# IanYeung/RealVSR

Hardware: AMD Instinct MI355X
Metric: HR frames/sec (fwd+bwd) on 5-frame 180x320 LR windows (higher is better)
Workload: dtype f32 (bf16x3 GEMM); 1 GPU; EDVR-M nf64, 5-frame 180x320 LR windows, batch 8 per GPU, x4 output, VideoSRModel.optimize_parameters: fwd + LapPyr(ssim,cb) on Y + GWLoss on CbCr + bwd + Adam step; per_gpu_batch=8, global_batch=8, parallelism=sequence-dp1, gemm=bf16x3 (3-term bf16 split on v_mfma_f32_32x32x16_bf16, f32 accumulate), lf_term=ssim (restated IQA_pytorch.SSIM, parity unpinned)

## Files before the change

include/realvsr_hip.h:

```cpp
#ifndef REALVSR_HIP_H
#define REALVSR_HIP_H
#include <stddef.h>
#ifdef __cplusplus
extern "C" {
#endif

#define RVSR_OK 0
#define RVSR_ERR_UNSUPPORTED 1
#define RVSR_ERR_BAD_ARG 2
#define RVSR_ERR_LAUNCH 3
#define RVSR_ERR_WORKSPACE 4

const char* rvsr_last_error(void);

void rvsr_set_gemm_mode(int mode);
int rvsr_get_gemm_mode(void);
void rvsr_set_gemm_mode_thread(int mode);


size_t rvsr_modulated_deform_conv_forward_workspace_bytes(int channels, int channels_out);
int rvsr_modulated_deform_conv_forward(const float* input, const float* weight, const float* bias,
                                       const float* offset, const float* mask, float* output,
                                       int batch, int channels, int height, int width, int channels_out,
                                       int kernel_h, int kernel_w, int stride_h, int stride_w,
// ... 44 lines not shown
int rvsr_dcn_pack_forward_plan(const float* input, const float* weight, const float* bias, const float* om,
                               float* output, int batch, int channels, int height, int width, int channels_out,
                               int stride, int pad, int dilation, int deformable_group, int act, float slope,
                               void* probe, void* workspace, size_t workspace_bytes, long long* plan);
int rvsr_dcn_pack_backward_plan(const float* input, const float* weight, const float* om, const float* grad_output,
                                const float* act_out, float act_slope, float* grad_input, float* grad_weight,
                                float* grad_bias, float* grad_om, int batch, int channels, int height, int width,
                                int channels_out, int stride, int pad, int dilation, int deformable_group,
                                const void* probe, void* workspace, size_t workspace_bytes, long long* plan);
int rvsr_dcn_fused_takes(int batch, int channels, int height, int width, int channels_out, int kernel_h, int kernel_w, int stride_h,
                         int stride_w, int pad_h, int pad_w, int dilation_h, int dilation_w, int group, int deformable_group);
size_t rvsr_dcn_probe_samples(int batch, int deformable_group, int height_out, int width_out);
int rvsr_dcn_forward_halo(const unsigned* counters, size_t nsamples, int channels_out);

size_t rvsr_deform_conv_generic_workspace_bytes(int dtype, int channels, int height, int width, int kernel_h, int kernel_w,
                                                int stride_h, int stride_w, int pad_h, int pad_w, int dilation_h, int dilation_w);
size_t rvsr_deform_conv_generic_forward_workspace_bytes(int dtype, int channels, int height, int width, int kernel_h, int kernel_w,
                                                        int stride_h, int stride_w, int pad_h, int pad_w, int dilation_h,
                                                        int dilation_w);
int rvsr_deform_conv_generic_forward(int dtype, const void* input, const void* weight, const void* bias, const void* offset,
                                     const void* mask, void* output, int batch, int channels, int height, int width,
                                     int channels_out, int kernel_h, int kernel_w, int stride_h, int stride_w, int pad_h, int pad_w,
                                     int dilation_h, int dilation_w, int group, int deformable_group, void* workspace,
                                     size_t workspace_bytes, void* stream);
int rvsr_deform_conv_generic_backward(int dtype, const void* input, const void* weight, const void* offset, const void* mask,
                                      const void* grad_output, void* grad_input, void* grad_offset, void* grad_mask,
                                      void* grad_weight, void* grad_bias, int batch, int channels, int height, int width,
                                      int channels_out, int kernel_h, int kernel_w, int stride_h, int stride_w, int pad_h, int pad_w,
                                      int dilation_h, int dilation_w, int group, int deformable_group, void* workspace,
                                      size_t workspace_bytes, void* stream);


size_t rvsr_conv2d_forward_workspace_bytes(int C1, int C2, int Co, int ksize);
int rvsr_conv2d_forward(const float* x1, int C1, const float* x2, int C2, const float* xact, float xact_slope,
                        int in_mode, int Hs, int Ws, const float* weight, const float* bias,
                        const float* residual, float* out1, int Co1, float* out2, int Co2, int B, int ksize,
                        int stride, int w_mode, int act, float slope, int pixel_shuffle, int Hout, int Wout,
                        void* workspace, size_t workspace_bytes, void* stream);
int rvsr_conv2d_forward_plan(const float* x1, int C1, const float* x2, int C2, const float* xact, float xact_slope,
                             int in_mode, int Hs, int Ws, const float* weight, const float* bias,
                             const float* residual, float* out1, int Co1, float* out2, int Co2, int B, int ksize,
                             int stride, int w_mode, int act, float slope, int pixel_shuffle, int Hout, int Wout, int* plan);

size_t rvsr_conv2d_pack_weights(const float* weight, int C_in, int Co, int ksize, int w_mode, void* out, size_t out_bytes,
                                long long* desc, void* stream);
int rvsr_pack_weights_batched(const void* descs, int n, void* stream);

size_t rvsr_conv2d_wgrad_workspace_bytes(int C1, int C2, int Co, int B, int ksize, int stride, int Hout, int Wout);
int rvsr_conv2d_backward_weight(const float* x1, int C1, const float* x2, int C2, int Hin, int Win,
                                const float* gout, const float* gact, float gact_slope, int g_mode,
                                int Gs_h, int Gs_w, float* grad_weight, float* grad_bias, int Co, int B,
                                int ksize, int stride, int Hout, int Wout, int accumulate,
                                void* workspace, size_t workspace_bytes, void* stream);


int rvsr_upsample_bilinear_forward(const float* in, float* out, size_t planes, int H, int W, int factor,
                                   float scale, void* stream);
int rvsr_upsample_bilinear_backward(const float* gout, float* gin, size_t planes, int H, int W, int factor,
                                    float scale, void* stream);

int rvsr_maxavgpool_forward(const float* in, float* out, unsigned char* argmax, int B, int C, int H, int W,
                            void* stream);
int rvsr_maxavgpool_backward(const float* gout, const unsigned char* argmax, float* gin, int B, int C, int H,
                             int W, void* stream);

int rvsr_tsa_temporal_forward(const float* emb, const float* emb_ref, const float* aligned, float* mod,
                              float* prob, int B, int N, int C, int H, int W, int frame_major, void* stream);
int rvsr_tsa_temporal_backward(const float* gmod, const float* emb, const float* emb_ref, const float* aligned,
                               const float* prob, float* galigned, float* gemb, float* gemb_ref, int B, int N,
                               int C, int H, int W, int frame_major, void* stream);

int rvsr_tsa_output_forward(const float* fea, const float* att, const float* att_add, float* out, size_t n,
                            void* stream);
int rvsr_tsa_output_backward(const float* g, const float* fea, const float* att, float* gfea, float* gatt,
                             size_t n, void* stream);


int rvsr_pyr_down_forward(const float* in, float* out, size_t planes, int H, int W, void* stream);
int rvsr_pyr_down_backward(const float* gout, float* gin, size_t planes, int H, int W, void* stream);
int rvsr_pyr_updiff_forward(const float* cur, const float* down, float* out, size_t planes, int H, int W,
                            void* stream);
int rvsr_pyr_updiff_backward(const float* gout, float* gdown, size_t planes, int H, int W, void* stream);

size_t rvsr_charbonnier_workspace_bytes(void);
int rvsr_charbonnier_forward(const float* x, const float* y, size_t n, float eps, double scale, float* out,
                             void* workspace, void* stream);
int rvsr_charbonnier_backward(const float* x, const float* y, const float* gscalar, float scale, float eps,
                              float* gx, size_t n, void* stream);

int rvsr_gwloss_forward(const float* x1, const float* x2, size_t planes, int H, int W, float w, double scale, float* out,
                        float* fa, float* fbx, float* fby, void* workspace, void* stream);
int rvsr_gwloss_backward(const float* fa, const float* fbx, const float* fby, const float* gscalar, float scale, float* gx,
                         size_t planes, int H, int W, void* stream);


int rvsr_ycbcr_to_bgr_u8(const float* ycc, unsigned char* bgr, int H, int W, void* stream);


size_t rvsr_reduce_workspace_bytes(void);

int rvsr_pixel_loss_forward(const float* x, const float* y, size_t n, int mode, float param, double scale, float* out,
                            void* workspace, void* stream);
int rvsr_pixel_loss_backward(const float* x, const float* y, const float* gscalar, int mode, float param, float scale,
                             float* gx, size_t n, void* stream);

int rvsr_ssim_forward(const float* x, const float* y, size_t planes, int H, int W, double scale, float* out, float* ga,
// ... 41 lines not shown
```

realvsr_amd/_lib.py:

```python
import ctypes
import os
import subprocess

import torch

_CSRC = os.path.join(os.path.dirname(os.path.abspath(__file__)), 'csrc')
SO_PATH = os.environ.get('RVSR_SO', os.path.join(_CSRC, 'librealvsr_hip.so'))
_lib = None

c_fp = ctypes.c_void_p
c_int, c_float, c_double, c_size = ctypes.c_int, ctypes.c_float, ctypes.c_double, ctypes.c_size_t

_CONV_CALL = [c_fp, c_int, c_fp, c_int, c_fp, c_float, c_int, c_int, c_int, c_fp, c_fp, c_fp, c_fp, c_int, c_fp, c_int, c_int, c_int,
              c_int, c_int, c_int, c_float, c_int, c_int, c_int]
SIGNATURES = {
    'rvsr_last_error': (ctypes.c_char_p, []),
    'rvsr_modulated_deform_conv_forward': (c_int, [c_fp] * 6 + [c_int] * 16 + [c_fp, c_size, c_fp]),
    'rvsr_modulated_deform_conv_forward_workspace_bytes': (c_size, [c_int] * 2),
    'rvsr_modulated_deform_conv_backward_workspace_bytes': (c_size, [c_int] * 8),
    'rvsr_modulated_deform_conv_backward': (c_int, [c_fp] * 11 + [c_int] * 16 + [c_fp, c_size, c_fp]),
    'rvsr_deform_conv_workspace_bytes': (c_size, [c_int] * 11),
    'rvsr_deform_conv_forward': (c_int, [c_fp] * 4 + [c_int] * 16 + [c_fp, c_size, c_fp]),
    'rvsr_deform_conv_backward_input': (c_int, [c_fp] * 6 + [c_int] * 16 + [c_fp, c_size, c_fp]),
    'rvsr_deform_conv_backward_parameters': (c_int, [c_fp] * 4 + [c_int] * 15 + [c_float, c_int, c_fp, c_size, c_fp]),
    'rvsr_deform_conv_generic_workspace_bytes': (c_size, [c_int] * 12),
    'rvsr_deform_conv_generic_forward_workspace_bytes': (c_size, [c_int] * 12),
    'rvsr_deform_conv_generic_forward': (c_int, [c_int] + [c_fp] * 6 + [c_int] * 15 + [c_fp, c_size, c_fp]),
    'rvsr_deform_conv_generic_backward': (c_int, [c_int] + [c_fp] * 10 + [c_int] * 15 + [c_fp, c_size, c_fp]),
    'rvsr_dcn_pack_forward': (c_int, [c_fp] * 5 + [c_int] * 10 + [c_float, c_fp, c_fp, c_size, c_fp]),
    'rvsr_dcn_offset_probe': (c_int, [c_fp, c_int, c_int, c_int, c_int, c_fp, c_fp]),
    'rvsr_dcn_pack_backward': (c_int, [c_fp] * 5 + [c_float] + [c_fp] * 4 + [c_int] * 9 + [c_fp, c_fp, c_size, c_fp]),
    'rvsr_dcn_pack_forward_plan': (c_int, [c_fp] * 5 + [c_int] * 10 + [c_float, c_fp, c_fp, c_size, ctypes.POINTER(ctypes.c_longlong)]),
    'rvsr_dcn_pack_backward_plan': (c_int, [c_fp] * 5 + [c_float] + [c_fp] * 4 + [c_int] * 9 + [c_fp, c_fp, c_size,
                                                                                             ctypes.POINTER(ctypes.c_longlong)]),
    'rvsr_dcn_fused_takes': (c_int, [c_int] * 15),
    'rvsr_dcn_probe_samples': (c_size, [c_int] * 4),
    'rvsr_dcn_forward_halo': (c_int, [c_fp, c_size, c_int]),
    'rvsr_conv2d_forward': (c_int, _CONV_CALL + [c_fp, c_size, c_fp]),
    'rvsr_conv2d_forward_plan': (c_int, _CONV_CALL + [ctypes.POINTER(c_int)]),
    'rvsr_conv2d_forward_workspace_bytes': (c_size, [c_int] * 4),
    'rvsr_conv2d_pack_weights': (c_size, [c_fp, c_int, c_int, c_int, c_int, c_fp, c_size, ctypes.POINTER(ctypes.c_longlong), c_fp]),
    'rvsr_dcn_pack_weights': (c_size, [c_fp, c_int, c_int, c_fp, c_size, ctypes.POINTER(ctypes.c_longlong), c_fp]),
    'rvsr_pack_weights_batched': (c_int, [c_fp, c_int, c_fp]),
    'rvsr_set_gemm_mode': (None, [c_int]),
    'rvsr_get_gemm_mode': (c_int, []),
    'rvsr_set_gemm_mode_thread': (None, [c_int]),
    'rvsr_conv2d_wgrad_workspace_bytes': (c_size, [c_int] * 8),
    'rvsr_conv2d_backward_weight': (c_int, [c_fp, c_int, c_fp, c_int, c_int, c_int, c_fp, c_fp, c_float, c_int, c_int,
                                            c_int, c_fp, c_fp, c_int, c_int, c_int, c_int, c_int, c_int, c_int, c_fp,
                                            c_size, c_fp]),
    'rvsr_upsample_bilinear_forward': (c_int, [c_fp, c_fp, c_size, c_int, c_int, c_int, c_float, c_fp]),
    'rvsr_upsample_bilinear_backward': (c_int, [c_fp, c_fp, c_size, c_int, c_int, c_int, c_float, c_fp]),
    'rvsr_maxavgpool_forward': (c_int, [c_fp, c_fp, c_fp, c_int, c_int, c_int, c_int, c_fp]),
    'rvsr_maxavgpool_backward': (c_int, [c_fp, c_fp, c_fp, c_int, c_int, c_int, c_int, c_fp]),
    'rvsr_tsa_temporal_forward': (c_int, [c_fp] * 5 + [c_int] * 6 + [c_fp]),
    'rvsr_tsa_temporal_backward': (c_int, [c_fp] * 8 + [c_int] * 6 + [c_fp]),
    'rvsr_tsa_output_forward': (c_int, [c_fp] * 4 + [c_size, c_fp]),
    'rvsr_tsa_output_backward': (c_int, [c_fp] * 5 + [c_size, c_fp]),
    'rvsr_pyr_down_forward': (c_int, [c_fp, c_fp, c_size, c_int, c_int, c_fp]),
    'rvsr_pyr_down_backward': (c_int, [c_fp, c_fp, c_size, c_int, c_int, c_fp]),
    'rvsr_pyr_updiff_forward': (c_int, [c_fp, c_fp, c_fp, c_size, c_int, c_int, c_fp]),
    'rvsr_pyr_updiff_backward': (c_int, [c_fp, c_fp, c_size, c_int, c_int, c_fp]),
    'rvsr_charbonnier_workspace_bytes': (c_size, []),
    'rvsr_charbonnier_forward': (c_int, [c_fp, c_fp, c_size, c_float, c_double, c_fp, c_fp, c_fp]),
    'rvsr_charbonnier_backward': (c_int, [c_fp, c_fp, c_fp, c_float, c_float, c_fp, c_size, c_fp]),
    'rvsr_gwloss_forward': (c_int, [c_fp, c_fp, c_size, c_int, c_int, c_float, c_double, c_fp, c_fp, c_fp, c_fp, c_fp, c_fp]),
    'rvsr_gwloss_backward': (c_int, [c_fp, c_fp, c_fp, c_fp, c_float, c_fp, c_size, c_int, c_int, c_fp]),
    'rvsr_ycbcr_to_bgr_u8': (c_int, [c_fp, c_fp, c_int, c_int, c_fp]),
    'rvsr_reduce_workspace_bytes': (c_size, []),
    'rvsr_pixel_loss_forward': (c_int, [c_fp, c_fp, c_size, c_int, c_float, c_double, c_fp, c_fp, c_fp]),
    'rvsr_pixel_loss_backward': (c_int, [c_fp, c_fp, c_fp, c_int, c_float, c_float, c_fp, c_size, c_fp]),
    'rvsr_ssim_forward': (c_int, [c_fp, c_fp, c_size, c_int, c_int, c_double, c_fp, c_fp, c_fp, c_fp, c_fp, c_fp]),
    'rvsr_ssim_backward': (c_int, [c_fp] * 6 + [c_float, c_fp, c_size, c_int, c_int, c_fp]),
    'rvsr_conv_gauss_forward': (c_int, [c_fp, c_fp, c_size, c_int, c_int, c_float, c_fp]),
    'rvsr_conv_gauss_backward': (c_int, [c_fp, c_fp, c_size, c_int, c_int, c_float, c_fp]),
    'rvsr_pyr_upsample_forward': (c_int, [c_fp, c_fp, c_size, c_int, c_int, c_fp]),
    'rvsr_pyr_upsample_backward': (c_int, [c_fp, c_fp, c_size, c_int, c_int, c_fp]),
    'rvsr_adam_step': (c_int, [c_fp] * 4 + [c_size] + [c_float] * 6 + [c_fp]),
    'rvsr_bcast_add_act': (c_int, [c_fp, c_fp, c_size, c_int, c_int, c_float, c_fp]),
    'rvsr_bcast_reduce_act': (c_int, [c_fp, c_fp, c_fp, c_size, c_int, c_float, c_fp]),
    'rvsr_augment_clips': (c_int, [c_fp] * 5 + [c_size] + [c_int] * 10 + [c_float, c_fp]),
    'rvsr_bn_workspace_bytes': (c_size, [c_int] * 3),
    'rvsr_bn_lrelu_forward': (c_int, [c_fp] * 9 + [c_int] * 4 + [c_float] * 3 + [c_fp, c_size, c_fp]),
    'rvsr_bn_lrelu_backward': (c_int, [c_fp] * 9 + [c_int] * 4 + [c_float, c_fp, c_size, c_fp]),
    'rvsr_gan_loss_forward': (c_int, [c_fp, c_size, c_fp, c_size, c_float, c_double, c_fp, c_fp, c_fp]),
    'rvsr_gan_loss_backward': (c_int, [c_fp, c_size, c_size, c_fp, c_fp, c_float, c_float, c_fp, c_fp, c_fp]),
    'rvsr_debug_mfma_rate': (c_int, [c_fp, c_fp, c_int, c_int, c_fp]),
}


def _p(t):
    return None if t is None else ctypes.c_void_p(t.data_ptr())


def _stream():
    return ctypes.c_void_p(torch.cuda.current_stream().cuda_stream)


def build(verbose=False):
    cmd = ['make', '-C', _CSRC, '-j4'] + ([] if verbose else ['-s'])
    subprocess.check_call(cmd)
    if not os.path.exists(SO_PATH):
        raise RuntimeError('build did not produce %s' % SO_PATH)
# ... 57 lines not shown
```

realvsr_amd/csrc/conv2_kernels.hip:

```cpp
#define RVSR_DEFINE_PACK
#include "conv_plan.h"

#include "bf16x3.h"

#ifdef RVSR_ABL5
constexpr int ABL5 = RVSR_ABL5;
#else
constexpr int ABL5 = 0;
#endif

#ifdef RVSR_TIMELINE
__device__ unsigned long long rvsr_dbg[512];
extern "C" int rvsr_debug_read(unsigned long long* out) { return (int)hipMemcpyFromSymbol(out, HIP_SYMBOL(rvsr_dbg), sizeof(unsigned long long) * 512); }
#define STAMP(i) do { if (blockIdx.x == 77 && tid == 0) rvsr_dbg[(i)] = __builtin_amdgcn_s_memtime(); } while (0)
#else
#define STAMP(i) do {} while (0)
#endif

template <int MT, int MODE>
__device__ __forceinline__ void conv2_epilogue(f32x16 (&acc)[MT][2], const ConvFwdParams& p, const float* bias_s, int b,
                                               int o0, int row0, int col, int hi) {
    const float neg = p.act == 0 ? 1.f : (p.act == 1 ? 0.f : p.slope);
    const bool col_ok = col < p.Wout;
    const size_t HW = (size_t)p.Hout * p.Wout;
// ... 1301 lines not shown
            g4[2 * s2] = *reinterpret_cast<const float4*>(gp + pc);
            g4[2 * s2 + 1] = *reinterpret_cast<const float4*>(gp + pc + 4);
            x4[2 * s2] = *reinterpret_cast<const float4*>(xp + pc);
            x4[2 * s2 + 1] = *reinterpret_cast<const float4*>(xp + pc + 4);
            if (ACT) {
                a4[2 * s2] = *reinterpret_cast<const float4*>(ap + pc);
                a4[2 * s2 + 1] = *reinterpret_cast<const float4*>(ap + pc + 4);
            }
        }
#pragma unroll
        for (int s2 = 0; s2 < 2; ++s2) {
            float gv[8] = {g4[2 * s2].x, g4[2 * s2].y, g4[2 * s2].z, g4[2 * s2].w,
                           g4[2 * s2 + 1].x, g4[2 * s2 + 1].y, g4[2 * s2 + 1].z, g4[2 * s2 + 1].w};
            float xv[8] = {x4[2 * s2].x, x4[2 * s2].y, x4[2 * s2].z, x4[2 * s2].w,
                           x4[2 * s2 + 1].x, x4[2 * s2 + 1].y, x4[2 * s2 + 1].z, x4[2 * s2 + 1].w};
            if (ACT) {
                const float av[8] = {a4[2 * s2].x, a4[2 * s2].y, a4[2 * s2].z, a4[2 * s2].w,
                                     a4[2 * s2 + 1].x, a4[2 * s2 + 1].y, a4[2 * s2 + 1].z, a4[2 * s2 + 1].w};
#pragma unroll
                for (int j = 0; j < 8; ++j) gv[j] *= av[j] > 0.f ? 1.f : p.g.slope;
            }
            const bool gok = pv[s2] && o_ok, xok = pv[s2] && c_ok;
#pragma unroll
            for (int j = 0; j < 8; ++j) {
                gv[j] = gok ? gv[j] : 0.f;
                xv[j] = xok ? xv[j] : 0.f;
                bsum += gv[j];
            }
            bf16x8 gh, gl, xh, xl;
            split8(gv, gh, gl);
            split8(xv, xh, xl);
            acc = mfma_bf16(gh, xh, acc);
            acc = mfma_bf16(gh, xl, acc);
            acc = mfma_bf16(gl, xh, acc);
        }
    }
    float* part = p.part + (size_t)blockIdx.x * p.Co * Ctot;
#pragma unroll
    for (int r = 0; r < 16; ++r) {
        const int orow = blockIdx.y * 64 + m * 32 + drow(r, hi);
        if (orow < p.Co && c_ok) part[(size_t)orow * Ctot + c] = acc[r];
    }
    if (p.bpart != nullptr && blockIdx.z == 0 && n == 0) {
        bsum += __shfl_xor(bsum, 32);
        if (hi == 0 && o_ok) p.bpart[(size_t)blockIdx.x * p.Co + o] = bsum;
    }
}

int rvsr_launch_conv_wgrad1x1(const ConvWgradParams& p, int gy, int gz, hipStream_t st) {
    auto k = p.g.act != nullptr ? conv_wgrad1x1_kernel<true> : conv_wgrad1x1_kernel<false>;
    return rvsr_conv_launch("conv_wgrad1x1", k, dim3(p.P, gy, gz), 256, 0, st, p);
}

template <bool ACT>
__global__ __launch_bounds__(256, 2) void conv_wgrad_s2_kernel(const ConvWgradParams p) {
    const int tid = threadIdx.x, lane = tid & 63, wave = tid >> 6, lo = lane & 31, hi = lane >> 5;
    const int m = wave & 1, n = wave >> 1;
    const int C = p.x.a.C;
    const int Hin = p.x.a.Hs, Win = p.x.a.Ws;
    const int Ho = p.Hout, Wo = p.Wout;
    const int o = blockIdx.y * 64 + m * 32 + lo;
    const int c = blockIdx.z * 64 + n * 32 + lo;
    const bool o_ok = o < p.Co, c_ok = c < C;
    const int oc = o_ok ? o : 0, cc = c_ok ? c : 0;
    const int UW = (Wo + 15) / 16;
    const long units = (long)p.B * Ho * UW;
    const long per = (units + p.P - 1) / p.P;
    long u0 = (long)blockIdx.x * per, u1 = u0 + per;
    if (u1 > units) u1 = units;
    f32x16 acc[9];
#pragma unroll
    for (int t = 0; t < 9; ++t) acc[t] = zero16();
    float bsum = 0.f;
    for (long u = u0; u < u1; ++u) {
        const int b = (int)(u / ((long)Ho * UW));
        const int rem = (int)(u - (long)b * Ho * UW);
        const int py = rem / UW, px0 = (rem - py * UW) * 16 + 8 * hi;
        const bool pv = px0 < Wo;
        const size_t gidx = (((size_t)b * p.Co + oc) * Ho + py) * Wo + (pv ? px0 : 0);
        const float4 g0 = *reinterpret_cast<const float4*>(p.g.p + gidx), g1 = *reinterpret_cast<const float4*>(p.g.p + gidx + 4);
        float4 a0, a1;
        if (ACT) {
            a0 = *reinterpret_cast<const float4*>(p.g.act + gidx);
            a1 = *reinterpret_cast<const float4*>(p.g.act + gidx + 4);
        }
        float xr[3][20];
#pragma unroll
        for (int dy = 0; dy < 3; ++dy) {
            const int iy = 2 * py + dy - 1;
            const bool rok = pv && c_ok && iy >= 0 && iy < Hin;
            const float* row = p.x.a.p + (((size_t)b * C + cc) * Hin + (rok ? iy : 0)) * Win;
#pragma unroll
            for (int j = 0; j < 5; ++j) {
                const int col = 2 * px0 - 4 + 4 * j;
                const bool ok = rok && col >= 0 && col < Win;
                const float4 q = *reinterpret_cast<const float4*>(row + (ok ? col : 0));
                xr[dy][4 * j + 0] = ok ? q.x : 0.f; xr[dy][4 * j + 1] = ok ? q.y : 0.f;
                xr[dy][4 * j + 2] = ok ? q.z : 0.f; xr[dy][4 * j + 3] = ok ? q.w : 0.f;
            }
        }
        float gv[8] = {g0.x, g0.y, g0.z, g0.w, g1.x, g1.y, g1.z, g1.w};
        if (ACT) {
            const float av[8] = {a0.x, a0.y, a0.z, a0.w, a1.x, a1.y, a1.z, a1.w};
#pragma unroll
            for (int j = 0; j < 8; ++j) gv[j] *= av[j] > 0.f ? 1.f : p.g.slope;
        }
// ... 148 lines not shown
```

realvsr_amd/csrc/conv_common.h:

```cpp
#pragma once
#include "rvsr_common.h"

struct ConvFwdParams {
    TCat in;
    const float* w;
    const void* wpack;
    int swz;
    int vec4;
    const float* bias;
    const float* res;
    float* out1;
    float* out2;
    int Co1;
    int B, Co, Hout, Wout;
    int w_mode;
    int prepacked;
    int fmt;
    int act;
    float slope;
    int ps;
    int ntx;
};


// ... 16 lines not shown
            for (int r = 0; r < 16; ++r) {
                const int o = o0 + m * 32 + 4 * hi + (r & 3) + 8 * (r >> 2);
                const bool ok = col_ok && o < p.Co;
                const int oc = ok ? o : 0;
                float v = acc[m][n][r];
                const float bb = bp[oc];
                v += has_bias ? bb : 0.f;
                v = v > 0.f ? v : v * neg;
                if (MODE == 3) {
                    const size_t idx = (((size_t)b * (p.Co >> 2) + (oc >> 2)) * (2 * p.Hout) + 2 * row + ((oc >> 1) & 1)) *
                                           (2 * p.Wout) + 2 * col + (oc & 1);
                    if (ok) p.out1[idx] = v;
                } else if (MODE == 2) {
                    const bool first = oc < p.Co1;
                    float* dst = first ? p.out1 : p.out2;
                    const size_t idx = ((size_t)b * (first ? p.Co1 : p.Co - p.Co1) + (first ? oc : oc - p.Co1)) * HW + pix;
                    if (ok) dst[idx] = v;
                } else {
                    const size_t idx = ((size_t)b * p.Co + oc) * HW + pix;
                    if (ok) {
                        if (MODE == 1) v += p.res[idx];
                        p.out1[idx] = v;
                    }
                }
            }
        }
    }
}


struct ConvWgradParams {
    TCat x;
    TView g;
    float* part;
    float* bpart;
    int B, Co, Hout, Wout, ntx, nty, P;
    int ring;
};


struct ConvFwdPlan;
template <typename K, typename P>
static inline int rvsr_conv_launch(const char* name, K k, dim3 grid, unsigned threads, size_t lds, hipStream_t st, const P& p) {
    if (set_lds(k, lds)) FAIL(RVSR_ERR_LAUNCH, "%s: cannot reserve %zu B of LDS", name, lds);
    hipLaunchKernelGGL(k, grid, dim3(threads), lds, st, p);
    hipError_t e = hipGetLastError();
    if (e != hipSuccess) FAIL(RVSR_ERR_LAUNCH, "%s launch: %s", name, hipGetErrorString(e));
    return RVSR_OK;
}
size_t rvsr_conv_fwd2_workspace_bytes(int ksize, int Co, int Ctot);
int rvsr_launch_conv_fwd2(ConvFwdParams p, const ConvFwdPlan& q, int ksize, int stride, void* workspace, size_t workspace_bytes, hipStream_t st);
int rvsr_launch_conv_wgrad2(const ConvWgradParams& p, int gy, int gz, hipStream_t st);
int rvsr_launch_conv_wgrad1x1(const ConvWgradParams& p, int gy, int gz, hipStream_t st);
int rvsr_launch_conv_wgrad_s2(const ConvWgradParams& p, int gy, int gz, hipStream_t st);
int rvsr_launch_conv_wgrad5(const ConvWgradParams& p, int stride, int gy, int gz, hipStream_t st);
int rvsr_launch_conv_wgrad_thin(const ConvWgradParams& p, hipStream_t st);
int rvsr_launch_conv_fwd_thin(const ConvFwdParams& p, const ConvFwdPlan& q, hipStream_t st);
```

realvsr_amd/csrc/conv_kernels.hip:

```cpp
#include "rvsr_common.h"

#include "conv_plan.h"

template <int KS, int STRIDE, int MT, int CC>
__global__ __launch_bounds__(RVSR_WG, 2) void conv_fwd_kernel(const ConvFwdParams p) {
    constexpr int T = KS * KS, PAD = KS / 2, TH = 8, TW = 32;
    constexpr int IH = (TH - 1) * STRIDE + KS, IW = (TW - 1) * STRIDE + KS;
    constexpr int MP = MT * 32, MPP = MP + 1;
    extern __shared__ __attribute__((aligned(16))) float smem[];
    float* xs = smem;
    float* ws = smem + CC * IH * IW;
    const int tid = threadIdx.x, lane = tid & 63, wave = tid >> 6, lo = lane & 31, hi = lane >> 5;
    const int tx = blockIdx.x % p.ntx, ty = blockIdx.x / p.ntx;
    const int x0 = tx * TW, y0 = ty * TH, mb = blockIdx.y, b = blockIdx.z;
    const int Ctot = p.in.a.C + p.in.b.C;

    f32x16 acc[MT][2];
#pragma unroll
    for (int m = 0; m < MT; ++m) {
        acc[m][0] = zero16();
        acc[m][1] = zero16();
    }

    for (int c0 = 0; c0 < Ctot; c0 += CC) {
// ... 302 lines not shown
                                   const float* bias, const float* residual, float* out1, int Co1, float* out2,
                                   int Co2, int B, int ksize, int stride, int w_mode, int act, float slope,
                                   int pixel_shuffle, int Hout, int Wout, void* workspace, size_t workspace_bytes,
                                   void* stream) {
    ConvFwdParams p;
    const int rc = conv_fwd_params(p, x1, C1, x2, C2, xact, xact_slope, in_mode, Hs, Ws, weight, bias, residual, out1, Co1, out2, Co2, B,
                                   ksize, stride, w_mode, act, slope, pixel_shuffle, Hout, Wout);
    if (rc) return rc;
    const ConvFwdPlan q = conv_fwd_plan(p, ksize, stride, rvsr_gemm_mode_now());
    if (q.rc) return conv_fwd_refuse(q);
    hipStream_t st = (hipStream_t)stream;
    switch (q.family) {
        case CONV_FWD_THIN: return rvsr_launch_conv_fwd_thin(p, q, st);
        case CONV_FWD_F32: return launch_fwd(p, q, ksize, stride, st);
        default: return rvsr_launch_conv_fwd2(p, q, ksize, stride, workspace, workspace_bytes, st);
    }
}
extern "C" int rvsr_conv2d_forward_plan(const float* x1, int C1, const float* x2, int C2, const float* xact,
                                        float xact_slope, int in_mode, int Hs, int Ws, const float* weight,
                                        const float* bias, const float* residual, float* out1, int Co1, float* out2,
                                        int Co2, int B, int ksize, int stride, int w_mode, int act, float slope,
                                        int pixel_shuffle, int Hout, int Wout, int* plan) {
    ConvFwdParams p;
    const int rc = conv_fwd_params(p, x1, C1, x2, C2, xact, xact_slope, in_mode, Hs, Ws, weight, bias, residual, out1, Co1, out2, Co2, B,
                                   ksize, stride, w_mode, act, slope, pixel_shuffle, Hout, Wout);
    if (rc) return rc;
    const ConvFwdPlan q = conv_fwd_plan(p, ksize, stride, rvsr_gemm_mode_now());
    const int row[14] = {q.family, q.mt, q.vec, q.wide, q.nt, q.act_in, q.cc, q.vec4, q.th, q.tw, (int)q.gx, (int)q.gy, (int)q.gz, (int)q.lds};
    for (int i = 0; plan && i < 14; ++i) plan[i] = row[i];
    return q.rc ? conv_fwd_refuse(q) : RVSR_OK;
}

int rvsr_g_gemm_mode = 0;
thread_local int rvsr_t_gemm_mode = -1;
extern "C" void rvsr_set_gemm_mode(int mode) { rvsr_g_gemm_mode = (mode >= 0 && mode <= 3) ? mode : 0; }
extern "C" void rvsr_set_gemm_mode_thread(int mode) { rvsr_t_gemm_mode = (mode >= 0 && mode <= 3) ? mode : -1; }
extern "C" int rvsr_get_gemm_mode() { return rvsr_gemm_mode_now(); }
extern "C" size_t rvsr_conv2d_forward_workspace_bytes(int C1, int C2, int Co, int ksize) {
    return rvsr_conv_fwd2_workspace_bytes(ksize, Co, C1 + C2);
}

extern "C" size_t rvsr_conv2d_wgrad_workspace_bytes(int C1, int C2, int Co, int B, int ksize, int stride, int Hout,
                                                    int Wout) {
    const size_t P = conv_wgrad_max_P(ksize, stride, B, Hout, Wout, Co, C1 + C2);
    return sizeof(float) * P * ((size_t)Co * (C1 + C2) * ksize * ksize + Co);
}

template <int KS, int STRIDE, int CCW>
static int launch_wgrad(const ConvWgradParams& p, int gy, int gz, hipStream_t st) {
    constexpr int IH = 3 * STRIDE + KS, IW = 31 * STRIDE + KS, CS = (IH * IW) | 1;
    return rvsr_conv_launch("conv_wgrad", conv_wgrad_kernel<KS, STRIDE, CCW>, dim3(p.P, gy, gz), RVSR_WG, sizeof(float) * (128 * 65 + CCW * CS), st, p);
}

extern "C" int rvsr_conv2d_backward_weight(const float* x1, int C1, const float* x2, int C2, int Hin, int Win,
                                           const float* gout, const float* gact, float gact_slope, int g_mode,
                                           int Gs_h, int Gs_w, float* grad_weight, float* grad_bias, int Co, int B,
                                           int ksize, int stride, int Hout, int Wout, int accumulate, void* workspace,
                                           size_t workspace_bytes, void* stream) {
    if (!x1 || !gout || !grad_weight || B <= 0) FAIL(RVSR_ERR_BAD_ARG, "conv2d_backward_weight: null/empty argument");
    if ((x2 == nullptr) != (C2 == 0)) FAIL(RVSR_ERR_BAD_ARG, "conv2d_backward_weight: x2/C2 disagree");
    if (ksize != 1 && ksize != 3 && ksize != 5) FAIL(RVSR_ERR_UNSUPPORTED, "conv2d_backward_weight: kernel size %d", ksize);
    if (stride != 1 && !(stride == 2 && ksize != 1)) FAIL(RVSR_ERR_UNSUPPORTED, "conv2d_backward_weight: stride %d", stride);
    if (g_mode != 0 && g_mode != 2) FAIL(RVSR_ERR_UNSUPPORTED, "conv2d_backward_weight: gradient view mode %d", g_mode);
    const size_t need = rvsr_conv2d_wgrad_workspace_bytes(C1, C2, Co, B, ksize, stride, Hout, Wout);
    if (!workspace || workspace_bytes < need)
        FAIL(RVSR_ERR_WORKSPACE, "conv2d_backward_weight: workspace %zu B < %zu B", workspace_bytes, need);
    ConvWgradParams p;
    make_view(p.x.a, x1, nullptr, 0.f, C1, Hin, Win, 0, 0, 0);
    make_view(p.x.b, x2, nullptr, 0.f, C2, Hin, Win, 0, 0, 0);
    if (make_view(p.g, gout, gact, gact_slope, Co, Gs_h, Gs_w, g_mode, 0, 0) || p.g.Hv != Hout || p.g.Wv != Wout)
        FAIL(RVSR_ERR_BAD_ARG, "conv2d_backward_weight: gradient view %dx%d (mode %d) vs output %dx%d", Gs_h, Gs_w, g_mode,
             Hout, Wout);
    const int pad = ksize / 2;
    if ((Hin + 2 * pad - ksize) / stride + 1 != Hout || (Win + 2 * pad - ksize) / stride + 1 != Wout)
        FAIL(RVSR_ERR_BAD_ARG, "conv2d_backward_weight: input %dx%d does not give output %dx%d", Hin, Win, Hout, Wout);
    p.B = B;
    p.Co = Co;
    p.Hout = Hout;
    p.Wout = Wout;
    p.ntx = (Wout + 31) / 32;
    p.nty = (Hout + 3) / 4;
    p.ring = 0;
    const ConvWgradPlan q = conv_wgrad_plan(p, ksize, stride, rvsr_gemm_mode_now());
    const size_t nw = (size_t)Co * (C1 + C2) * ksize * ksize;
    p.P = q.P;
    p.part = (float*)workspace;
    p.bpart = grad_bias ? p.part + (size_t)p.P * nw : nullptr;
    hipStream_t st = (hipStream_t)stream;
    int rc = RVSR_ERR_UNSUPPORTED;
    switch (q.family) {
        case CONV_WGRAD_THIN: rc = rvsr_launch_conv_wgrad_thin(p, st); break;
        case CONV_WGRAD2: rc = rvsr_launch_conv_wgrad2(p, q.gy, q.gz, st); break;
        case CONV_WGRAD5: rc = rvsr_launch_conv_wgrad5(p, stride, q.gy, q.gz, st); break;
        case CONV_WGRAD_F32_5: rc = stride == 1 ? launch_wgrad<5, 1, 16>(p, q.gy, q.gz, st) : launch_wgrad<5, 2, 16>(p, q.gy, q.gz, st); break;
        case CONV_WGRAD_1X1: rc = rvsr_launch_conv_wgrad1x1(p, q.gy, q.gz, st); break;
        case CONV_WGRAD_F32_3S1: rc = launch_wgrad<3, 1, 64>(p, q.gy, q.gz, st); break;
        case CONV_WGRAD_S2: rc = rvsr_launch_conv_wgrad_s2(p, q.gy, q.gz, st); break;
        case CONV_WGRAD_F32_3S2: rc = launch_wgrad<3, 2, 32>(p, q.gy, q.gz, st); break;
        case CONV_WGRAD_F32_1: rc = launch_wgrad<1, 1, 64>(p, q.gy, q.gz, st); break;
    }
    if (rc) return rc;
    rvsr_launch_reduce(p.part, p.P, nw, grad_weight, accumulate, st, p.bpart, (size_t)Co, grad_bias);
    hipError_t e = hipGetLastError();
    if (e != hipSuccess) FAIL(RVSR_ERR_LAUNCH, "conv_wgrad reduce launch: %s", hipGetErrorString(e));
    return RVSR_OK;
}
```

realvsr_amd/csrc/conv_plan.h:

```cpp
#pragma once
#include "conv_common.h"

static inline bool conv_al16(const void* a, const void* b = nullptr, const void* c = nullptr, const void* d = nullptr) {
    return ((((uintptr_t)a) | ((uintptr_t)b) | ((uintptr_t)c) | ((uintptr_t)d)) & 15) == 0;
}
static inline bool conv_span_ok(size_t H, size_t W, size_t C) { return sizeof(float) * H * W * C < ((size_t)1 << 31); }


enum ConvFwdFamily {
    CONV_FWD_THIN = 0,
    CONV_FWD5 = 1,
    CONV_FWD2 = 2,
    CONV_FWD_F32 = 3,
};

struct ConvFwdPlan {
    int rc;
    const char* msg;
    int family;
    int mt;
    int vec;
    int wide;
    int nt;
    int act_in;
// ... 70 lines not shown
        q.cc = ksize == 1 ? 32 : ksize == 3 ? (stride == 1 ? (wide_m ? 8 : 16) : (wide_m ? 4 : 8)) : (stride == 1 ? (wide_m ? 4 : 8) : 4);
        const int IH = 7 * stride + ksize, IW = 31 * stride + ksize;
        q.lds = sizeof(float) * ((size_t)q.cc * IH * IW + (size_t)T * q.cc * (q.mt * 32 + 1));
        q.gx = (unsigned)(ntx * nty8);
        q.gy = (unsigned)((p.Co + q.mt * 32 - 1) / (q.mt * 32));
        q.gz = (unsigned)p.B;
        return q;
    }
    q.vec4 = (p.Wout % 4 == 0) && conv_al16(p.out1, p.res) && !p.ps && p.out2 == nullptr && conv_span_ok(p.Hout, p.Wout, p.Co);
    q.cc = ccg;
    q.gy = q.gz = 1;
    long items = (long)nmb * p.B;
    if (ksize != 3 || stride != 1) {
        q.family = CONV_FWD2;
        const int IH = 7 * stride + ksize, IW = 31 * stride + ksize;
        q.lds = (size_t)16 * (2 * (2 * ccg) * IH * IW + 2 * T * (2 * ccg) * (q.mt * 32)) + sizeof(float) * q.mt * 32;
        items *= (long)ntx * nty8;
        const int slots = 256 * (q.lds > 80 * 1024 ? 1 : 2);
        q.gx = (unsigned)(items < slots ? items : slots);
        return q;
    }
    q.family = CONV_FWD5;
    const bool al = conv_al16(va.p, va.act, vb.p);
    if (va.mode == 0 && va.Ws % 4 == 0 && va.Wv == va.Ws && al && conv_span_ok(va.Hs, va.Ws, va.C > vb.C ? va.C : vb.C) &&
        (vb.C == 0 || va.C % 16 == 0))
        q.vec = 1;
    else if (va.mode == 2 && vb.C == 0 && va.C % 16 == 0 && va.Wv % 4 == 0 && va.Ws == 2 * va.Wv && va.Hs == 2 * va.Hv && al &&
             conv_span_ok(va.Hs, va.Ws, va.C >> 2))
        q.vec = 2;
    else if (va.mode == 1 && vb.C == 0 && va.Wv % 4 == 0 && va.Wv == 2 * va.Ws && va.Hv <= 2 * va.Hs && va.Ws % 2 == 0 && al &&
             conv_span_ok(va.Hs, va.Ws, va.C))
        q.vec = 3;
    if (p.fmt && (q.vec != 1 || q.act_in))
        return conv_fwd_refusal("conv2d: the f16 + fp8 format needs a plain 16-byte-aligned input view with W % 4 == 0 and no act' tensor");
    const long px_n = (long)((p.Hout + 15) / 16 * 16) * ((p.Wout + 31) / 32 * 32), px_w = (long)((p.Hout + 7) / 8 * 8) * ((p.Wout + 63) / 64 * 64);
    q.wide = q.mt == 2 && q.vec == 1 && q.vec4 && px_w <= px_n;
    if (p.act == 3 && !q.wide) return conv_fwd_refusal(nullptr);
    if (p.fmt) q.nt = 4;
    else if (q.mt == 2 && q.vec != 0) q.nt = gemm_mode == 2 ? 2 : (gemm_mode == 3 ? 1 : 3);
    q.th = q.wide ? 8 : 16;
    q.tw = q.wide ? 64 : 32;
    const int NX = q.wide ? 2 * 10 * 66 : 2 * 18 * 34, WVEC = 9 * 2 * q.mt * 32;
    q.lds = (size_t)16 * (2 * 2 * NX + 2 * 2 * WVEC) + sizeof(float) * 4 * q.mt * 32 + 16;
    items *= (long)((p.Wout + q.tw - 1) / q.tw) * ((p.Hout + q.th - 1) / q.th);
    q.gx = (unsigned)(items < 256 ? items : 256);
    return q;
}

enum ConvWgradFamily {
    CONV_WGRAD_THIN = 0,
    CONV_WGRAD2,
    CONV_WGRAD5,
    CONV_WGRAD_F32_5,
    CONV_WGRAD_1X1,
    CONV_WGRAD_F32_3S1,
    CONV_WGRAD_S2,
    CONV_WGRAD_F32_3S2,
    CONV_WGRAD_F32_1,
    CONV_WGRAD_FAMILIES
};
struct ConvWgradPlan {
    int family, P, gy, gz;
};

static inline bool conv_wgrad_can(int family, int ksize, int stride, int Co) {
    switch (family) {
        case CONV_WGRAD_THIN: return ksize == 3 && stride == 1 && Co <= 4;
        case CONV_WGRAD2: case CONV_WGRAD_F32_3S1: return ksize == 3 && stride == 1;
        case CONV_WGRAD5: case CONV_WGRAD_F32_5: return ksize == 5;
        case CONV_WGRAD_S2: case CONV_WGRAD_F32_3S2: return ksize == 3 && stride == 2;
        default: return ksize == 1;
    }
}
static inline ConvWgradPlan conv_wgrad_slicing(int family, int B, int Hout, int Wout, int Co, int Ctot) {
    const long ntiles = (long)B * ((Hout + 3) / 4) * ((Wout + 31) / 32);
    long units = ntiles, slots = 256;
    int gy = (Co + 63) / 64, gz = (Ctot + 63) / 64;
    switch (family) {
        case CONV_WGRAD_THIN:
            units = (long)B * ((Hout + 3) / 4) * ((Wout + 63) / 64);
            slots = 768;
            gy = gz = 1;
            break;
        case CONV_WGRAD5:
            gy = (Co + 31) / 32;
            gz = (Ctot + 31) / 32;
            break;
        case CONV_WGRAD_F32_5:
            gz = (Ctot + 15) / 16;
            break;
        case CONV_WGRAD_S2:
            units = (long)B * Hout * ((Wout + 15) / 16);
            slots = 512;
            break;
        case CONV_WGRAD_F32_3S2:
            gz = (Ctot + 31) / 32;
            break;
        case CONV_WGRAD_1X1: case CONV_WGRAD_F32_1:
            slots = 1024;
            break;
        default:
            break;
    }
    long P = slots / ((long)gy * gz);
    if (P < 1) P = 1;
    if (P > units) P = units;
    return {family, (int)P, gy, gz};
}
static inline int conv_wgrad_max_P(int ksize, int stride, int B, int Hout, int Wout, int Co, int Ctot) {
    int P = 0;
    for (int f = 0; f < CONV_WGRAD_FAMILIES; ++f)
        if (conv_wgrad_can(f, ksize, stride, Co)) {
            const int Pf = conv_wgrad_slicing(f, B, Hout, Wout, Co, Ctot).P;
            if (Pf > P) P = Pf;
        }
    return P;
}

static inline ConvWgradPlan conv_wgrad_plan(const ConvWgradParams& p, int ksize, int stride, int gemm_mode) {
    const int C1 = p.x.a.C, C2 = p.x.b.C, Ctot = C1 + C2;
    const bool al = conv_al16(p.x.a.p, p.x.b.p, p.g.p, p.g.act), split = gemm_mode != 1, plain_g = p.g.mode == 0;
    const auto takes = [&](int family) {
        switch (family) {
            case CONV_WGRAD_THIN:
                return C2 == 0 && C1 % 16 == 0 && plain_g && p.Wout % 4 == 0 && al && conv_span_ok(p.Hout, p.Wout, C1);
            case CONV_WGRAD2:
                return split && p.Wout % 4 == 0 && al && conv_span_ok(p.Hout, p.Wout, p.Co > Ctot ? p.Co : Ctot) && (C2 == 0 || C1 % 64 == 0);
            case CONV_WGRAD5: return split;
            case CONV_WGRAD_1X1: return split && plain_g && (p.Hout * p.Wout) % 8 == 0 && al;
            case CONV_WGRAD_S2: return split && C2 == 0 && plain_g && p.Wout % 8 == 0 && p.x.a.Ws % 4 == 0 && al;
            default: return true;
        }
    };
    for (int f = 0; f < CONV_WGRAD_FAMILIES; ++f)
        if (conv_wgrad_can(f, ksize, stride, p.Co) && takes(f)) return conv_wgrad_slicing(f, p.B, p.Hout, p.Wout, p.Co, Ctot);
    return {-1, 0, 0, 0};
}
```

Measured before the change: 81.42 HR frames/s.

## Add wide-channel 1x1 weight-gradient kernel with LDS staging and prefetch

Adds a 512-thread 1x1 conv weight-gradient kernel. Each block covers 64 output channels by up to 320 input channels, stages bf16 hi/lo splits of the gradient and input tiles in LDS, and prefetches the next pixel tile through buffer loads while the current one runs bf16x3 MFMAs. It is placed ahead of the existing 1x1 family in the planner, with its own slicing rules, and a plan-query API is exposed. The aim is more reuse of each gradient tile across many input channels and loads hidden behind compute. In exchange, occupancy drops to one block per CU and there are fewer partial slices to reduce.

Result: faster. 82.26 HR frames/s, median of 6 (+1.0%).

```diff
diff --git a/include/realvsr_hip.h b/include/realvsr_hip.h
--- a/include/realvsr_hip.h
+++ b/include/realvsr_hip.h
@@ -120,6 +120,10 @@
                                 int Gs_h, int Gs_w, float* grad_weight, float* grad_bias, int Co, int B,
                                 int ksize, int stride, int Hout, int Wout, int accumulate,
                                 void* workspace, size_t workspace_bytes, void* stream);
+int rvsr_conv2d_backward_weight_plan(const float* x1, int C1, const float* x2, int C2, int Hin, int Win,
+                                     const float* gout, const float* gact, float gact_slope, int g_mode,
+                                     int Gs_h, int Gs_w, float* grad_weight, int Co, int B, int ksize, int stride,
+                                     int Hout, int Wout, int* plan);
 
 
 int rvsr_upsample_bilinear_forward(const float* in, float* out, size_t planes, int H, int W, int factor,
diff --git a/realvsr_amd/_lib.py b/realvsr_amd/_lib.py
--- a/realvsr_amd/_lib.py
+++ b/realvsr_amd/_lib.py
@@ -49,6 +49,8 @@
     'rvsr_conv2d_backward_weight': (c_int, [c_fp, c_int, c_fp, c_int, c_int, c_int, c_fp, c_fp, c_float, c_int, c_int,
                                             c_int, c_fp, c_fp, c_int, c_int, c_int, c_int, c_int, c_int, c_int, c_fp,
                                             c_size, c_fp]),
+    'rvsr_conv2d_backward_weight_plan': (c_int, [c_fp, c_int, c_fp, c_int, c_int, c_int, c_fp, c_fp, c_float, c_int, c_int, c_int, c_fp] +
+                                         [c_int] * 6 + [ctypes.POINTER(c_int)]),
     'rvsr_upsample_bilinear_forward': (c_int, [c_fp, c_fp, c_size, c_int, c_int, c_int, c_float, c_fp]),
     'rvsr_upsample_bilinear_backward': (c_int, [c_fp, c_fp, c_size, c_int, c_int, c_int, c_float, c_fp]),
     'rvsr_maxavgpool_forward': (c_int, [c_fp, c_fp, c_fp, c_int, c_int, c_int, c_int, c_fp]),
diff --git a/realvsr_amd/csrc/conv2_kernels.hip b/realvsr_amd/csrc/conv2_kernels.hip
--- a/realvsr_amd/csrc/conv2_kernels.hip
+++ b/realvsr_amd/csrc/conv2_kernels.hip
@@ -1377,6 +1377,158 @@
     return rvsr_conv_launch("conv_wgrad1x1", k, dim3(p.P, gy, gz), 256, 0, st, p);
 }
 
+#define WG1_THREADS 512
+#define WG1_KT 64
+#define WG1_CB 320
+#define WG1_RP 144
+#define WG1_ROWS (64 + WG1_CB)
+template <bool ACT>
+__global__ __launch_bounds__(WG1_THREADS, 1) void conv_wgrad1x1s_kernel(const ConvWgradParams p) {
+    extern __shared__ __attribute__((aligned(16))) unsigned char smem_raw[];
+    unsigned char* t_hi = smem_raw;
+    unsigned char* t_lo = smem_raw + WG1_ROWS * WG1_RP;
+    const int tid = threadIdx.x, lane = tid & 63, wave = tid >> 6, lo = lane & 31, hi = lane >> 5;
+    const int m = wave & 1, ng = wave >> 1;
+    const int C1 = p.x.a.C, C2 = p.x.b.C, Ctot = C1 + C2;
+    const int HW = p.Hout * p.Wout;
+    const int o0 = blockIdx.y * 64, c0 = blockIdx.z * WG1_CB;
+    const int cb = Ctot - c0 < WG1_CB ? Ctot - c0 : WG1_CB;
+    const int nblk = (cb + 63) / 64, ntile = (cb + 31) / 32;
+    const bool m_live = o0 + m * 32 < p.Co;
+    const bool do_bias = p.bpart != nullptr && blockIdx.z == 0;
+
+    constexpr int NXI = WG1_CB / 64;
+    constexpr unsigned OOB = 0x80000000u;
+    const int q = tid & 7, r64 = tid >> 3;
+    const unsigned g_vo = o0 + r64 < p.Co ? 4u * (unsigned)((o0 + r64) * HW + 8 * q) : OOB;
+    unsigned x_vo[NXI];
+#pragma unroll
+    for (int i = 0; i < NXI; ++i) {
+        const int c = c0 + 64 * i + r64;
+        x_vo[i] = c < Ctot ? 4u * (unsigned)((c >= C1 ? c - C1 : c) * HW + 8 * q) : OOB;
+    }
+    const size_t img_g = (size_t)p.Co * HW, img_x1 = (size_t)C1 * HW, img_x2 = (size_t)C2 * HW;
+
+    typedef float f32x4v __attribute__((ext_vector_type(4)));
+    auto ld4 = [&](__amdgpu_buffer_rsrc_t rs, unsigned vo, unsigned so) {
+        const f32x4v v = __builtin_bit_cast(f32x4v, __builtin_amdgcn_raw_buffer_load_b128(rs, (int)vo, (int)so, 0));
+        return make_float4(v.x, v.y, v.z, v.w);
+    };
+    float4 gv[2], sv[ACT ? 2 : 1], xv[NXI][2];
+    float bacc = 0.f;
+
+    const int U = (HW + WG1_KT - 1) / WG1_KT;
+    const int ntiles = p.B * U;
+    const int per = (ntiles + p.P - 1) / p.P;
+    const int t_begin = blockIdx.x * per, t_end = t_begin + per < ntiles ? t_begin + per : ntiles;
+
+    auto issue_loads = [&](int tile, int part) {
+        int b = tile / U;
+        int px0 = (tile - b * U) * WG1_KT;
+        asm volatile("" : "+s"(b), "+s"(px0));
+        const int left = HW - px0;
+        const unsigned so = 4u * (unsigned)px0;
+        if (part < 0 || part == 0) {
+            const __amdgpu_buffer_rsrc_t g_rs = buf_view_2g(p.g.p + (size_t)b * img_g);
+            const __amdgpu_buffer_rsrc_t s_rs = buf_view_2g(ACT ? p.g.act + (size_t)b * img_g : p.g.p);
+#pragma unroll
+            for (int kk = 0; kk < 2; ++kk) {
+                const unsigned vo = 8 * q + 4 * kk < left ? g_vo + 16u * kk : OOB;
+                gv[kk] = ld4(g_rs, vo, so);
+                if (ACT) sv[kk] = ld4(s_rs, vo, so);
+            }
+        }
+#pragma unroll
+        for (int i = 0; i < NXI; ++i) {
+            if (part >= 0 && part != 1 + (i >> 1)) continue;
+            const bool sec = c0 + 64 * i >= C1;
+            const float* ximg = sec ? p.x.b.p + (size_t)b * img_x2 : p.x.a.p + (size_t)b * img_x1;
+            const __amdgpu_buffer_rsrc_t x_rs = buf_view_2g(c0 + 64 * i < Ctot ? ximg : p.x.a.p);
+#pragma unroll
+            for (int kk = 0; kk < 2; ++kk) xv[i][kk] = ld4(x_rs, 8 * q + 4 * kk < left ? x_vo[i] + 16u * kk : OOB, so);
+        }
+    };
+    auto commit = [&]() {
+        {
+            float v[8] = {gv[0].x, gv[0].y, gv[0].z, gv[0].w, gv[1].x, gv[1].y, gv[1].z, gv[1].w};
+            if (ACT) {
+                const float s[8] = {sv[0].x, sv[0].y, sv[0].z, sv[0].w, sv[1].x, sv[1].y, sv[1].z, sv[1].w};
+#pragma unroll
+                for (int j = 0; j < 8; ++j) v[j] *= s[j] > 0.f ? 1.f : p.g.slope;
+            }
+            bacc += ((v[0] + v[1]) + (v[2] + v[3])) + ((v[4] + v[5]) + (v[6] + v[7]));
+            bf16x8 h8, l8;
+            split8(v, h8, l8);
+            *reinterpret_cast<bf16x8*>(t_hi + r64 * WG1_RP + q * 16) = h8;
+            *reinterpret_cast<bf16x8*>(t_lo + r64 * WG1_RP + q * 16) = l8;
+        }
+#pragma unroll
+        for (int i = 0; i < NXI; ++i) {
+            if (i >= nblk) continue;
+            const float v[8] = {xv[i][0].x, xv[i][0].y, xv[i][0].z, xv[i][0].w, xv[i][1].x, xv[i][1].y, xv[i][1].z, xv[i][1].w};
+            bf16x8 h8, l8;
+            split8(v, h8, l8);
+            const int dst = (64 + 64 * i + r64) * WG1_RP + q * 16;
+            *reinterpret_cast<bf16x8*>(t_hi + dst) = h8;
+            *reinterpret_cast<bf16x8*>(t_lo + dst) = l8;
+        }
+    };
+
+    f32x16 acc[3];
+#pragma unroll
+    for (int j = 0; j < 3; ++j) acc[j] = zero16();
+    if (t_begin < t_end) issue_loads(t_begin, -1);
+    for (int tile = t_begin; tile < t_end; ++tile) {
+        const int next = tile + 1 < t_end ? tile + 1 : tile;
+        commit();
+        __syncthreads();
+#pragma unroll
+        for (int ks = 0; ks < WG1_KT / 16; ++ks) {
+            issue_loads(next, ks);
+            __builtin_amdgcn_sched_barrier(0);
+            if (!m_live) continue;
+            const int koff = ks * 32 + hi * 16;
+            const int goff = (m * 32 + lo) * WG1_RP + koff;
+            const bf16x8 ah = *reinterpret_cast<const bf16x8*>(t_hi + goff), al = *reinterpret_cast<const bf16x8*>(t_lo + goff);
+#pragma unroll
+            for (int j = 0; j < 3; ++j) {
+                const int nt = ng + 4 * j;
+                if (nt >= ntile) continue;
+                const int xoff = (64 + nt * 32 + lo) * WG1_RP + koff;
+                const bf16x8 bh = *reinterpret_cast<const bf16x8*>(t_hi + xoff), bl = *reinterpret_cast<const bf16x8*>(t_lo + xoff);
+                acc[j] = mfma_bf16(ah, bh, acc[j]);
+                acc[j] = mfma_bf16(ah, bl, acc[j]);
+                acc[j] = mfma_bf16(al, bh, acc[j]);
+            }
+        }
+        __syncthreads();
+    }
+
+    float* part = p.part + (size_t)blockIdx.x * p.Co * Ctot;
+#pragma unroll
+    for (int j = 0; j < 3; ++j) {
+        const int nt = ng + 4 * j, c = c0 + nt * 32 + lo;
+        if (!m_live || nt >= ntile || c >= Ctot) continue;
+#pragma unroll
+        for (int r = 0; r < 16; ++r) {
+            const int o = o0 + m * 32 + drow(r, hi);
+            if (o < p.Co) part[(size_t)o * Ctot + c] = acc[j][r];
+        }
+    }
+    if (do_bias) {
+        float v = bacc;
+        v += __shfl_xor(v, 1);
+        v += __shfl_xor(v, 2);
+        v += __shfl_xor(v, 4);
+        if (q == 0 && o0 + r64 < p.Co) p.bpart[(size_t)blockIdx.x * p.Co + o0 + r64] = v;
+    }
+}
+
+int rvsr_launch_conv_wgrad1x1s(const ConvWgradParams& p, int gy, int gz, hipStream_t st) {
+    auto k = p.g.act != nullptr ? conv_wgrad1x1s_kernel<true> : conv_wgrad1x1s_kernel<false>;
+    return rvsr_conv_launch("conv_wgrad1x1s", k, dim3(p.P, gy, gz), WG1_THREADS, (size_t)2 * WG1_ROWS * WG1_RP, st, p);
+}
+
 template <bool ACT>
 __global__ __launch_bounds__(256, 2) void conv_wgrad_s2_kernel(const ConvWgradParams p) {
     const int tid = threadIdx.x, lane = tid & 63, wave = tid >> 6, lo = lane & 31, hi = lane >> 5;
diff --git a/realvsr_amd/csrc/conv_common.h b/realvsr_amd/csrc/conv_common.h
--- a/realvsr_amd/csrc/conv_common.h
+++ b/realvsr_amd/csrc/conv_common.h
@@ -92,6 +92,7 @@
 int rvsr_launch_conv_fwd2(ConvFwdParams p, const ConvFwdPlan& q, int ksize, int stride, void* workspace, size_t workspace_bytes, hipStream_t st);
 int rvsr_launch_conv_wgrad2(const ConvWgradParams& p, int gy, int gz, hipStream_t st);
 int rvsr_launch_conv_wgrad1x1(const ConvWgradParams& p, int gy, int gz, hipStream_t st);
+int rvsr_launch_conv_wgrad1x1s(const ConvWgradParams& p, int gy, int gz, hipStream_t st);
 int rvsr_launch_conv_wgrad_s2(const ConvWgradParams& p, int gy, int gz, hipStream_t st);
 int rvsr_launch_conv_wgrad5(const ConvWgradParams& p, int stride, int gy, int gz, hipStream_t st);
 int rvsr_launch_conv_wgrad_thin(const ConvWgradParams& p, hipStream_t st);
diff --git a/realvsr_amd/csrc/conv_kernels.hip b/realvsr_amd/csrc/conv_kernels.hip
--- a/realvsr_amd/csrc/conv_kernels.hip
+++ b/realvsr_amd/csrc/conv_kernels.hip
@@ -378,20 +378,14 @@
     return rvsr_conv_launch("conv_wgrad", conv_wgrad_kernel<KS, STRIDE, CCW>, dim3(p.P, gy, gz), RVSR_WG, sizeof(float) * (128 * 65 + CCW * CS), st, p);
 }
 
-extern "C" int rvsr_conv2d_backward_weight(const float* x1, int C1, const float* x2, int C2, int Hin, int Win,
-                                           const float* gout, const float* gact, float gact_slope, int g_mode,
-                                           int Gs_h, int Gs_w, float* grad_weight, float* grad_bias, int Co, int B,
-                                           int ksize, int stride, int Hout, int Wout, int accumulate, void* workspace,
-                                           size_t workspace_bytes, void* stream) {
+static int conv_wgrad_params(ConvWgradParams& p, const float* x1, int C1, const float* x2, int C2, int Hin, int Win, const float* gout,
+                             const float* gact, float gact_slope, int g_mode, int Gs_h, int Gs_w, float* grad_weight, int Co, int B,
+                             int ksize, int stride, int Hout, int Wout) {
     if (!x1 || !gout || !grad_weight || B <= 0) FAIL(RVSR_ERR_BAD_ARG, "conv2d_backward_weight: null/empty argument");
     if ((x2 == nullptr) != (C2 == 0)) FAIL(RVSR_ERR_BAD_ARG, "conv2d_backward_weight: x2/C2 disagree");
     if (ksize != 1 && ksize != 3 && ksize != 5) FAIL(RVSR_ERR_UNSUPPORTED, "conv2d_backward_weight: kernel size %d", ksize);
     if (stride != 1 && !(stride == 2 && ksize != 1)) FAIL(RVSR_ERR_UNSUPPORTED, "conv2d_backward_weight: stride %d", stride);
     if (g_mode != 0 && g_mode != 2) FAIL(RVSR_ERR_UNSUPPORTED, "conv2d_backward_weight: gradient view mode %d", g_mode);
-    const size_t need = rvsr_conv2d_wgrad_workspace_bytes(C1, C2, Co, B, ksize, stride, Hout, Wout);
-    if (!workspace || workspace_bytes < need)
-        FAIL(RVSR_ERR_WORKSPACE, "conv2d_backward_weight: workspace %zu B < %zu B", workspace_bytes, need);
-    ConvWgradParams p;
     make_view(p.x.a, x1, nullptr, 0.f, C1, Hin, Win, 0, 0, 0);
     make_view(p.x.b, x2, nullptr, 0.f, C2, Hin, Win, 0, 0, 0);
     if (make_view(p.g, gout, gact, gact_slope, Co, Gs_h, Gs_w, g_mode, 0, 0) || p.g.Hv != Hout || p.g.Wv != Wout)
@@ -400,13 +394,44 @@
     const int pad = ksize / 2;
     if ((Hin + 2 * pad - ksize) / stride + 1 != Hout || (Win + 2 * pad - ksize) / stride + 1 != Wout)
         FAIL(RVSR_ERR_BAD_ARG, "conv2d_backward_weight: input %dx%d does not give output %dx%d", Hin, Win, Hout, Wout);
+    p.part = p.bpart = nullptr;
     p.B = B;
     p.Co = Co;
     p.Hout = Hout;
     p.Wout = Wout;
     p.ntx = (Wout + 31) / 32;
     p.nty = (Hout + 3) / 4;
+    p.P = 0;
     p.ring = 0;
+    return RVSR_OK;
+}
+
+extern "C" int rvsr_conv2d_backward_weight_plan(const float* x1, int C1, const float* x2, int C2, int Hin, int Win,
+                                                const float* gout, const float* gact, float gact_slope, int g_mode,
+                                                int Gs_h, int Gs_w, float* grad_weight, int Co, int B, int ksize, int stride,
+                                                int Hout, int Wout, int* plan) {
+    ConvWgradParams p;
+    const int rc = conv_wgrad_params(p, x1, C1, x2, C2, Hin, Win, gout, gact, gact_slope, g_mode, Gs_h, Gs_w, grad_weight, Co, B, ksize,
+                                     stride, Hout, Wout);
+    if (rc) return rc;
+    const ConvWgradPlan q = conv_wgrad_plan(p, ksize, stride, rvsr_gemm_mode_now());
+    const int row[4] = {q.family, q.P, q.gy, q.gz};
+    for (int i = 0; plan && i < 4; ++i) plan[i] = row[i];
+    return RVSR_OK;
+}
+
+extern "C" int rvsr_conv2d_backward_weight(const float* x1, int C1, const float* x2, int C2, int Hin, int Win,
+                                           const float* gout, const float* gact, float gact_slope, int g_mode,
+                                           int Gs_h, int Gs_w, float* grad_weight, float* grad_bias, int Co, int B,
+                                           int ksize, int stride, int Hout, int Wout, int accumulate, void* workspace,
+                                           size_t workspace_bytes, void* stream) {
+    ConvWgradParams p;
+    const int prc = conv_wgrad_params(p, x1, C1, x2, C2, Hin, Win, gout, gact, gact_slope, g_mode, Gs_h, Gs_w, grad_weight, Co, B, ksize,
+                                      stride, Hout, Wout);
+    if (prc) return prc;
+    const size_t need = rvsr_conv2d_wgrad_workspace_bytes(C1, C2, Co, B, ksize, stride, Hout, Wout);
+    if (!workspace || workspace_bytes < need)
+        FAIL(RVSR_ERR_WORKSPACE, "conv2d_backward_weight: workspace %zu B < %zu B", workspace_bytes, need);
     const ConvWgradPlan q = conv_wgrad_plan(p, ksize, stride, rvsr_gemm_mode_now());
     const size_t nw = (size_t)Co * (C1 + C2) * ksize * ksize;
     p.P = q.P;
@@ -419,6 +444,7 @@
         case CONV_WGRAD2: rc = rvsr_launch_conv_wgrad2(p, q.gy, q.gz, st); break;
         case CONV_WGRAD5: rc = rvsr_launch_conv_wgrad5(p, stride, q.gy, q.gz, st); break;
         case CONV_WGRAD_F32_5: rc = stride == 1 ? launch_wgrad<5, 1, 16>(p, q.gy, q.gz, st) : launch_wgrad<5, 2, 16>(p, q.gy, q.gz, st); break;
+        case CONV_WGRAD_1X1S: rc = rvsr_launch_conv_wgrad1x1s(p, q.gy, q.gz, st); break;
         case CONV_WGRAD_1X1: rc = rvsr_launch_conv_wgrad1x1(p, q.gy, q.gz, st); break;
         case CONV_WGRAD_F32_3S1: rc = launch_wgrad<3, 1, 64>(p, q.gy, q.gz, st); break;
         case CONV_WGRAD_S2: rc = rvsr_launch_conv_wgrad_s2(p, q.gy, q.gz, st); break;
diff --git a/realvsr_amd/csrc/conv_plan.h b/realvsr_amd/csrc/conv_plan.h
--- a/realvsr_amd/csrc/conv_plan.h
+++ b/realvsr_amd/csrc/conv_plan.h
@@ -146,6 +146,7 @@
     CONV_WGRAD2,
     CONV_WGRAD5,
     CONV_WGRAD_F32_5,
+    CONV_WGRAD_1X1S,
     CONV_WGRAD_1X1,
     CONV_WGRAD_F32_3S1,
     CONV_WGRAD_S2,
@@ -190,6 +191,15 @@
         case CONV_WGRAD_F32_3S2:
             gz = (Ctot + 31) / 32;
             break;
+        case CONV_WGRAD_1X1S: {
+            const long P1 = 1024 / ((long)gy * gz);
+            gz = (Ctot + 319) / 320;
+            units = (long)B * ((Hout * Wout + 63) / 64);
+            if (units > ntiles) units = ntiles;
+            slots = 256;
+            if (P1 < slots / ((long)gy * gz)) slots = P1 * gy * gz;
+            break;
+        }
         case CONV_WGRAD_1X1: case CONV_WGRAD_F32_1:
             slots = 1024;
             break;
@@ -221,6 +231,9 @@
             case CONV_WGRAD2:
                 return split && p.Wout % 4 == 0 && al && conv_span_ok(p.Hout, p.Wout, p.Co > Ctot ? p.Co : Ctot) && (C2 == 0 || C1 % 64 == 0);
             case CONV_WGRAD5: return split;
+            case CONV_WGRAD_1X1S:
+                return split && plain_g && (p.Hout * p.Wout) % 4 == 0 && al && (C2 == 0 || C1 % 64 == 0) &&
+                       conv_span_ok(p.Hout, p.Wout, p.Co > (C1 > C2 ? C1 : C2) ? p.Co : (C1 > C2 ? C1 : C2));
             case CONV_WGRAD_1X1: return split && plain_g && (p.Hout * p.Wout) % 8 == 0 && al;
             case CONV_WGRAD_S2: return split && C2 == 0 && plain_g && p.Wout % 8 == 0 && p.x.a.Ws % 4 == 0 && al;
             default: return true;
```
